# HilaManor/AudioEditingCode

Measured on AMD Instinct MI355X. Metric: edited-clips/sec (200-step inv+edit, 10 s@16 kHz), higher is better.
Workload: dtype f32

## Files before the change

audioeditingcode_amd/csrc/cg_params.h:

```cpp
#pragma once
#include "aed_common.h"

typedef float f32x16 __attribute__((ext_vector_type(16)));

struct CGParams {
    const float* A;
    const float* W;
    const float* bias;
    float* C;
    const float* res;
    const float* rowvec;
    float* ws;
    long long* dbg;
    const float* A2;
    int diag;
    int gm;
    int M, N, K;
    int lda, ldc, ldr, ld_rv;
    int IH, IW, OH, OW, Cin;
    int KH, KW, stride, pad_h, pad_w, dil_h, dil_w, up;
    int a_bs;
    int vIH, vIW;
    int o_mul, o_add, o_len, out_bs;
    int in_act, out_act, accumulate, ksplit;
    int rpb;
    int nchunks;
    int kgroup;
    float in_slope, out_p, out_div;
    int ln_mode;
    float ln_eps;
    int C1, lda2, a_bs2;
    int late_epilogue;
    int w_bs, vec_bs, vec_ld;
    int sm_group;
    float sm_scale;
    const float* kbias;
    int geglu;
    const unsigned char* Wq;
    const unsigned char* Wsc;
};

__device__ __forceinline__ float in_transform(float v, int act, float slope) {
    if (act == AED_ACT_SILU) return v / (1.0f + __expf(-v));
    if (act == AED_ACT_LEAKY) return v > 0.0f ? v : v * slope;
    return v;
}

__device__ __forceinline__ float gelu_exact(float g) { return 0.5f * g * (1.0f + erff(g * 0.70710678118654752440f)); }
__device__ __forceinline__ float glu_gate(float g, int kind) { return kind == 2 ? g / (1.0f + expf(-g)) : gelu_exact(g); }

__device__ __forceinline__ void store_out(const CGParams& p, int m, int n, float v) {
    int b = m / p.rpb;
    int q = m - b * p.rpb;
    int o = q * p.o_mul + p.o_add;
    if ((unsigned)o >= (unsigned)p.o_len) return;
    size_t row = (size_t)b * p.out_bs + o;
    if (p.bias) v += p.bias[n];
    if (p.rowvec && !p.ln_mode) v += p.rowvec[(size_t)b * p.ld_rv + n];
    if (p.res) v += p.res[row * p.ldr + n];
    v = aed_apply_act(v, p.out_act, p.out_p);
    float* dst = p.C + row * p.ldc + n;
    if (p.accumulate == 1) v += *dst;
    else if (p.accumulate == 2) v = (*dst + v) / p.out_div;
    *dst = v;
}

int cg_fill_params(const aed_op* op, CGParams& p, int bkt);
int launch_lin_gemm(const CGParams& p, int cfg, hipStream_t s);
```

audioeditingcode_amd/csrc/conv_gemm.hip:

```cpp
#include "cg_params.h"

template <int BM, int BN, int WROWS, int WCOLS, bool GENERIC, int DEPTH, int BKT, bool PLAIN>
__global__ __launch_bounds__(256, (BM * BN >= 128 * 128) ? 2 : 1) void conv_gemm_kernel(CGParams p) {
    constexpr int WM = BM / WROWS, WN = BN / WCOLS;
    constexpr int TM = WM / 32, TN = WN / 32;
    constexpr int LDS_LD = BKT + 4;
    constexpr int STAGE = (BM + BN) * LDS_LD;
    constexpr int TPR = BKT / 4;
    constexpr int RPP = 256 / TPR;
    constexpr int PA = BM / RPP, PB = BN / RPP;
    constexpr int NKB = BKT / 8;
    static_assert(WROWS * WCOLS == 4, "4 waves");
    static_assert(TM >= 1 && TN >= 1 && PA >= 1 && PB >= 1, "tile");

    __shared__ __attribute__((aligned(16))) float lds[2 * STAGE];

    const int tid = threadIdx.x;
    const int lane = tid & 63;
    const int wave = tid >> 6;
    const int wr = wave / WCOLS, wc = wave % WCOLS;
    int tile_x = blockIdx.x, tile_y = blockIdx.y;
    if (gridDim.z == 1) {
        const unsigned nx = gridDim.x, nwg = nx * gridDim.y;
        const unsigned orig = blockIdx.y * nx + blockIdx.x;
// ... 252 lines not shown
    if ((p.N & 3) == 0) {
        const size_t q4 = total >> 2;
        const float4* ws4 = reinterpret_cast<const float4*>(p.ws);
        for (size_t e4 = (size_t)blockIdx.x * 256 + threadIdx.x; e4 < q4; e4 += (size_t)gridDim.x * 256) {
            float4 v = ws4[e4];
#pragma unroll 4
            for (int z = 1; z < p.ksplit; ++z) {
                const float4 w = ws4[(size_t)z * q4 + e4];
                v.x += w.x; v.y += w.y; v.z += w.z; v.w += w.w;
            }
            const size_t e = e4 << 2;
            const int m = (int)(e / p.N);
            const int n = (int)(e - (size_t)m * p.N);
            store_out(p, m, n, v.x);
            store_out(p, m, n + 1, v.y);
            store_out(p, m, n + 2, v.z);
            store_out(p, m, n + 3, v.w);
        }
        return;
    }
    for (size_t e = (size_t)blockIdx.x * 256 + threadIdx.x; e < total; e += (size_t)gridDim.x * 256) {
        int m = (int)(e / p.N);
        int n = (int)(e - (size_t)m * p.N);
        float v = 0.f;
        for (int z = 0; z < p.ksplit; ++z) v += p.ws[(size_t)z * total + e];
        store_out(p, m, n, v);
    }
}

int cg_fill_params(const aed_op* op, CGParams& p, int bkt) {
    p.A = (const float*)op->p[0];
    p.W = (const float*)op->p[1];
    p.bias = (const float*)op->p[2];
    p.C = (float*)op->p[3];
    p.res = (const float*)op->p[4];
    p.rowvec = (const float*)op->p[5];
    p.ws = (float*)op->p[6];
    p.dbg = (op->flags & 1) ? (long long*)op->p[7] : nullptr;
    p.late_epilogue = (op->flags & 2) ? 1 : 0;
    const int32_t* i = op->i;
    p.M = i[0]; p.N = i[1]; p.K = i[2]; p.lda = i[3]; p.ldc = i[4]; p.ldr = i[5]; p.ld_rv = i[6];
    p.IH = i[7]; p.IW = i[8]; p.OH = i[9]; p.OW = i[10]; p.Cin = i[11]; p.KH = i[12]; p.KW = i[13];
    p.stride = i[14]; p.pad_h = i[15]; p.pad_w = i[16]; p.dil_h = i[17]; p.dil_w = i[18]; p.up = i[19];
    p.a_bs = i[20]; p.o_mul = i[21]; p.o_add = i[22]; p.o_len = i[23]; p.out_bs = i[24];
    p.in_act = i[25]; p.out_act = i[26]; p.accumulate = i[27]; p.ksplit = i[28];
    p.in_slope = op->f[0]; p.out_p = op->f[1]; p.out_div = op->f[2];
    p.ln_mode = i[31]; p.ln_eps = op->f[3];
    p.C1 = i[32]; p.lda2 = i[33]; p.a_bs2 = i[34]; p.geglu = i[35];
    p.A2 = (const float*)op->p[8];
    p.gm = 0;
    p.diag = (op->flags & 0x8000) ? 1 : 0;
    p.Wq = nullptr;
    p.Wsc = nullptr;
    p.sm_group = i[36]; p.w_bs = i[37]; p.vec_ld = i[38] > 0 ? i[38] : 1; p.vec_bs = i[39];
    p.sm_scale = op->f[4];
    p.kbias = (const float*)op->p[9];
    p.rpb = p.OH * p.OW;
    p.nchunks = (p.K + bkt - 1) / bkt;
    {
        const int g = bkt > 32 ? bkt : 32;
        p.kgroup = (p.KH * p.KW > 1 && p.Cin % g == 0 && p.Cin > g && !(op->flags & 32)) ? g : p.Cin;
    }
    p.vIH = p.IH << p.up;
    p.vIW = p.IW << p.up;
    if (p.up) {
        const int th = (p.OH - 1) * p.stride - 2 * p.pad_h + p.dil_h * (p.KH - 1) + 1;
        const int tw = (p.OW - 1) * p.stride - 2 * p.pad_w + p.dil_w * (p.KW - 1) + 1;
        if (th < p.vIH) p.vIH = th;
        if (tw < p.vIW) p.vIW = tw;
        AED_REQUIRE(p.vIH >= 2 * p.IH - 1 && p.vIW >= 2 * p.IW - 1, "conv_gemm: upsample target %dx%d too small for %dx%d",
                    th, tw, p.IH, p.IW);
    }
    AED_REQUIRE(p.A && p.W && p.C, "conv_gemm: null operand");
    AED_REQUIRE(p.M > 0 && p.N > 0 && p.K > 0, "conv_gemm: bad shape M=%d N=%d K=%d", p.M, p.N, p.K);
    AED_REQUIRE(p.K == p.KH * p.KW * p.Cin, "conv_gemm: K=%d != KH*KW*Cin=%d", p.K, p.KH * p.KW * p.Cin);
    AED_REQUIRE(p.rpb > 0 && p.M % p.rpb == 0, "conv_gemm: M=%d not a multiple of OH*OW=%d", p.M, p.rpb);
    AED_REQUIRE((long long)(p.M / p.rpb) * p.a_bs + (long long)p.IH * p.IW * p.lda < (1LL << 31) &&
                    (long long)p.N * p.K < (1LL << 31) &&
                    ((long long)(p.M / p.rpb) * p.out_bs + 1) * (long long)(p.ldc > p.ldr ? p.ldc : p.ldr) < (1LL << 31),
                "conv_gemm: operand exceeds the 32-bit element-offset range");
    if (p.ksplit < 1) p.ksplit = 1;
    if (p.ksplit > p.nchunks) p.ksplit = p.nchunks;
    if (p.ksplit > 1) AED_REQUIRE(p.ws != nullptr, "conv_gemm: split-K needs a workspace");
    if (p.ln_mode)
        AED_REQUIRE(p.ksplit == 1 && p.KH * p.KW == 1 && p.rowvec && p.bias && p.in_act == 0,
                    "conv_gemm: fused LayerNorm needs a 1-tap, unsplit GEMM with folded weights");
    if (p.C1 > 0)
        AED_REQUIRE(p.A2 && p.C1 % 64 == 0 && p.C1 < p.Cin && p.lda2 % 4 == 0 && ((uintptr_t)p.A2 % 16) == 0 &&
                        (long long)(p.M / p.rpb) * p.a_bs2 + (long long)p.IH * p.IW * p.lda2 < (1LL << 31),
                    "conv_gemm: bad two-source split C1=%d of Cin=%d", p.C1, p.Cin);
    if (p.geglu)
        AED_REQUIRE(p.ksplit == 1 && p.N % 64 == 0 && !p.res && p.out_act == 0 && p.accumulate == 0 && p.o_mul == 1 &&
                        p.o_add == 0 && p.o_len >= p.rpb && (p.ln_mode || !p.rowvec),
                    "conv_gemm: the GEGLU epilogue needs an unsplit GEMM with packed N %% 64 == 0 and a plain epilogue");
    return 0;
}

template <int BM, int BN, int WR, int WC, int DEPTH, int BKT>
static void launch_cfg(const CGParams& p, bool plain, hipStream_t s) {
    dim3 grid(aed_cdiv(p.N, BN), aed_cdiv(p.M, BM), p.ksplit);
    if (plain)
        hipLaunchKernelGGL((conv_gemm_kernel<BM, BN, WR, WC, false, DEPTH, BKT, true>), grid, dim3(256), 0, s, p);
    else
        hipLaunchKernelGGL((conv_gemm_kernel<BM, BN, WR, WC, false, DEPTH, BKT, false>), grid, dim3(256), 0, s, p);
}

// ... 83 lines not shown
```

audioeditingcode_amd/csrc/conv_gemm_x6.hip:

```cpp
#include "cg_params.h"

typedef __bf16 bf16x8 __attribute__((ext_vector_type(8)));
typedef __bf16 bf16x2 __attribute__((ext_vector_type(2)));
typedef float f32x2 __attribute__((ext_vector_type(2)));

int launch_conv_gemm_x6(const aed_op* op, hipStream_t s);

constexpr int X6_BK = 16;

__device__ __forceinline__ void x6_split_pair(float x0, float x1, unsigned& h, unsigned& m, unsigned& l) {
    h = __builtin_bit_cast(unsigned, __builtin_convertvector((f32x2){x0, x1}, bf16x2));
    float r0 = x0 - __uint_as_float(h << 16);
    float r1 = x1 - __uint_as_float(h & 0xffff0000u);
    asm volatile("" : "+v"(r0), "+v"(r1));
    m = __builtin_bit_cast(unsigned, __builtin_convertvector((f32x2){r0, r1}, bf16x2));
    float q0 = r0 - __uint_as_float(m << 16);
    float q1 = r1 - __uint_as_float(m & 0xffff0000u);
    asm volatile("" : "+v"(q0), "+v"(q1));
    l = __builtin_bit_cast(unsigned, __builtin_convertvector((f32x2){q0, q1}, bf16x2));
}

typedef unsigned u32x4 __attribute__((ext_vector_type(4)));
constexpr unsigned X6_OOB = 0x80000000u;

template <int G, int NM, int NV>
__device__ __forceinline__ void x6_hints() {
    if constexpr (G < NM) {
        constexpr int v = (NV * (G + 1)) / NM - (NV * G) / NM;
        if constexpr (v > 0) __builtin_amdgcn_sched_group_barrier(0x002, v, 0);
        __builtin_amdgcn_sched_group_barrier(0x008, 1, 0);
        x6_hints<G + 1, NM, NV>();
    }
}

template <int BM, int BN, int WROWS, int WCOLS, int DEPTH, bool PLAIN, int SCHED, int NTERMS, int BK = X6_BK>
__global__ __launch_bounds__(64 * WROWS * WCOLS, 2) void conv_gemm_x6_kernel(CGParams p) {
    constexpr int NT = 64 * WROWS * WCOLS;
    constexpr int WM = BM / WROWS, WN = BN / WCOLS;
    constexpr int TM = WM / 32, TN = WN / 32;
    constexpr int TPR = BK / 4;
    constexpr int RPP = NT / TPR;
    constexpr int PA = BM / RPP, PB = BN / RPP;
    constexpr int PQ = BK / 8;
    constexpr int X6_ROWQ = 3 * PQ + 1;
    constexpr int KB = BK / 16;
    constexpr int STAGE = (BM + BN) * X6_ROWQ;
    static_assert(BK == 16 || BK == 32, "chunk width");
    static_assert(TM >= 1 && TN >= 1 && PA >= 1 && PB >= 1, "tile");
    static_assert(BM % RPP == 0 && BN % RPP == 0, "loader passes");

    __shared__ uint4 lds[2 * STAGE];
    const unsigned nx = gridDim.x, ny = gridDim.y, bz = blockIdx.z, gz = gridDim.z;
    const unsigned orig = blockIdx.y * nx + blockIdx.x;

    const int tid = threadIdx.x;
    const int lane = tid & 63;
    const int wave = tid >> 6;
    const int wr = wave / WCOLS, wc = wave % WCOLS;
    int tile_y = (int)(orig / nx), tile_x = (int)(orig - (unsigned)tile_y * nx);
    if (gz == 1) {
        const unsigned nwg = nx * ny;
        const unsigned xcd = orig & 7u, q = nwg >> 3, r = nwg & 7u;
        const unsigned id = (xcd < r ? xcd * (q + 1) : r * (q + 1) + (xcd - r) * q) + (orig >> 3);
        if (p.gm > 1) {
            const unsigned per_group = (unsigned)p.gm * nx;
            const unsigned g = id / per_group, first = g * (unsigned)p.gm;
            const unsigned gsz = min((unsigned)p.gm, ny - first);
            const unsigned within = id - g * per_group;
            tile_x = (int)(within / gsz);
            tile_y = (int)(first + (within - (unsigned)tile_x * gsz));
        } else {
            tile_y = (int)(id / nx);
            tile_x = (int)(id - (unsigned)tile_y * nx);
        }
    }
    const int m0 = tile_y * BM;
    const int n0 = tile_x * BN;

    int kc_begin = 0, kc_end = p.nchunks;
    if (p.ksplit > 1) {
        const int per = (p.nchunks + p.ksplit - 1) / p.ksplit;
        kc_begin = (int)bz * per;
        kc_end = min(p.nchunks, kc_begin + per);
    }

    const int lrow = tid / TPR;
    const int lq = tid % TPR;
    const int lcol = lq * 4;

    int ay0[PA], ax0[PA];
    unsigned abase[PA], abase2[PA];
    bool avalid[PA];
#pragma unroll
    for (int q = 0; q < PA; ++q) {
        const int m = m0 + lrow + RPP * q;
        avalid[q] = m < p.M;
        const int mm = avalid[q] ? m : 0;
        int b = 0, r = mm, oy = mm, ox = 0;
        if (p.rpb != p.M || p.OW != 1) {
            b = mm / p.rpb;
            r = mm - b * p.rpb;
            oy = r / p.OW;
            ox = r - oy * p.OW;
        }
        ay0[q] = oy * p.stride - p.pad_h;
        ax0[q] = ox * p.stride - p.pad_w;
        abase[q] = (unsigned)b * (unsigned)p.a_bs + lcol;
        abase2[q] = (unsigned)b * (unsigned)p.a_bs2 + lcol;
    }
    unsigned wbase[PB];
    bool wvalid[PB];
#pragma unroll
    for (int q = 0; q < PB; ++q) {
        const int n = n0 + lrow + RPP * q;
        wvalid[q] = n < p.N;
        wbase[q] = (unsigned)(wvalid[q] ? n : 0) * (unsigned)p.K + lcol;
    }
    const int vIH = p.vIH, vIW = p.vIW;
    int pf_cg, pf_sub, pf_ty, pf_tx;
    const int gq = p.kgroup / BK;
    if (kc_begin == 0) {
        pf_cg = pf_sub = pf_ty = pf_tx = 0;
    } else {
        const int per_group = p.KH * p.KW * gq;
        const int g = kc_begin / per_group;
        const int rem = kc_begin - g * per_group;
        const int tap = rem / gq;
        pf_cg = g * p.kgroup;
        pf_sub = rem - tap * gq;
        pf_ty = tap / p.KW;
        pf_tx = tap - pf_ty * p.KW;
    }

    float4 rbuf_a[DEPTH][PA], rbuf_b[DEPTH][PB];
    float ln_s1[PA], ln_s2[PA];
#pragma unroll
    for (int q = 0; q < PA; ++q) { ln_s1[q] = 0.f; ln_s2[q] = 0.f; }

    const __amdgpu_buffer_rsrc_t srd_a = __builtin_amdgcn_make_buffer_rsrc((void*)p.A, 0, 0x7ffffff0, 0x00020000);
    const __amdgpu_buffer_rsrc_t srd_a2 = __builtin_amdgcn_make_buffer_rsrc((void*)(p.A2 ? p.A2 : p.A), 0, 0x7ffffff0, 0x00020000);
    const __amdgpu_buffer_rsrc_t srd_w = __builtin_amdgcn_make_buffer_rsrc((void*)p.W, 0, 0x7ffffff0, 0x00020000);
    auto as_f4 = [](u32x4 v) {
        return make_float4(__uint_as_float(v.x), __uint_as_float(v.y), __uint_as_float(v.z), __uint_as_float(v.w));
    };
    auto prefetch = [&](int kc, float4 (&ra)[PA], float4 (&rb)[PB]) {
        int c0 = pf_cg + pf_sub * BK;
        const int dy = pf_ty * p.dil_h, dx = pf_tx * p.dil_w;
        const unsigned k0 = (unsigned)((pf_ty * p.KW + pf_tx) * p.Cin + c0);
        pf_sub += 1;
        const bool wrap = pf_sub == gq;
        pf_sub = wrap ? 0 : pf_sub;
        pf_tx += wrap ? 1 : 0;
        const bool wrap2 = pf_tx == p.KW;
        pf_tx = wrap2 ? 0 : pf_tx;
        pf_ty += wrap2 ? 1 : 0;
        const bool wrap3 = pf_ty == p.KH;
        pf_ty = wrap3 ? 0 : pf_ty;
        pf_cg += wrap3 ? p.kgroup : 0;
        const bool second = p.C1 > 0 && c0 >= p.C1;
        c0 -= second ? p.C1 : 0;
        const unsigned ld = second ? (unsigned)p.lda2 : (unsigned)p.lda;
        const bool dead = kc >= kc_end;
#pragma unroll
        for (int q = 0; q < PA; ++q) {
            const int iy = ay0[q] + dy, ix = ax0[q] + dx;
            const bool ok = avalid[q] & ((unsigned)iy < (unsigned)vIH) & ((unsigned)ix < (unsigned)vIW) & !dead;
            const unsigned base = second ? abase2[q] : abase[q];
            const unsigned off = (base + (unsigned)((iy >> p.up) * p.IW + (ix >> p.up)) * ld + (unsigned)c0) * 4u;
            ra[q] = as_f4(__builtin_amdgcn_raw_buffer_load_b128(second ? srd_a2 : srd_a, ok ? off : X6_OOB, 0, 0));
        }
// ... 41 lines not shown
            }
            put_row(st, lrow + RPP * q, v);
        }
#pragma unroll
        for (int q = 0; q < PB; ++q) put_row(st, BM + lrow + RPP * q, rb[q], true);
    };

    f32x16 acc[TM][TN];
#pragma unroll
    for (int a = 0; a < TM; ++a)
#pragma unroll
        for (int b = 0; b < TN; ++b)
#pragma unroll
            for (int r = 0; r < 16; ++r) acc[a][b][r] = 0.f;

    const int fi = lane & 31;
    const int fh = lane >> 5;
    const int a_frag = (wr * WM + fi) * X6_ROWQ + fh;
    const int b_frag = (BM + wc * WN + fi) * X6_ROWQ + fh;

    bf16x8 af[TM][3], bw[TN][3];
    auto load_frags = [&](const uint4* st, int kb, bf16x8 (&fa)[TM][3], bf16x8 (&fb)[TN][3]) {
#pragma unroll
        for (int a = 0; a < TM; ++a)
#pragma unroll
            for (int pl = 0; pl < 3; ++pl)
                fa[a][pl] = __builtin_bit_cast(bf16x8, st[a_frag + a * 32 * X6_ROWQ + PQ * pl + 2 * kb]);
#pragma unroll
        for (int b = 0; b < TN; ++b)
#pragma unroll
            for (int pl = 0; pl < 3; ++pl)
                fb[b][pl] = __builtin_bit_cast(bf16x8, st[b_frag + b * 32 * X6_ROWQ + PQ * pl + 2 * kb]);
    };
    auto do_mfmas = [&](const bf16x8 (&fa)[TM][3], const bf16x8 (&fb)[TN][3]) {
        constexpr int TA[6] = {0, 2, 1, 0, 1, 0};
        constexpr int TB[6] = {2, 0, 1, 1, 0, 0};
#pragma unroll
        for (int t = 6 - NTERMS; t < 6; ++t)
#pragma unroll
            for (int a = 0; a < TM; ++a)
#pragma unroll
                for (int b = 0; b < TN; ++b)
                    acc[a][b] = __builtin_amdgcn_mfma_f32_32x32x16_bf16(fa[a][TA[t]], fb[b][TB[t]], acc[a][b], 0, 0, 0);
    };
    auto hints = [&]() {
        if constexpr (SCHED == 1) {
            constexpr int NM = TM * TN * NTERMS * KB;
            x6_hints<0, NM, NM * (((PA + PB) * 22 + 40 + NM - 1) / NM)>();
        }
    };

#pragma unroll
    for (int d = 0; d < DEPTH; ++d) prefetch(kc_begin + d, rbuf_a[d], rbuf_b[d]);
    stage_write(lds, rbuf_a[0], rbuf_b[0]);
    prefetch(kc_begin + DEPTH, rbuf_a[0], rbuf_b[0]);
    __syncthreads();
    int cur = 0;
    for (int kc0 = kc_begin; kc0 < kc_end; kc0 += DEPTH) {
#pragma unroll
        for (int d = 0; d < DEPTH; ++d) {
            const int kc = kc0 + d;
            const int sl = (d + 1) % DEPTH;
            load_frags(lds + cur * STAGE, 0, af, bw);
            stage_write(lds + (cur ^ 1) * STAGE, rbuf_a[sl], rbuf_b[sl]);
            prefetch(kc + 1 + DEPTH, rbuf_a[sl], rbuf_b[sl]);
            do_mfmas(af, bw);
            if constexpr (KB == 2) {
                bf16x8 af2[TM][3], bw2[TN][3];
                load_frags(lds + cur * STAGE, 1, af2, bw2);
                do_mfmas(af2, bw2);
            }
            hints();
            __syncthreads();
            cur ^= 1;
        }
    }

    float* ln_stat = reinterpret_cast<float*>(lds);
#include "cg_epilogue.h"
}

template <int BM, int BN, int WR, int WC, int DEPTH, bool DIAG, int BK = X6_BK>
static int x6_launch(const CGParams& p, bool plain, int sched, int terms, hipStream_t s) {
    dim3 grid(aed_cdiv(p.N, BN), aed_cdiv(p.M, BM), p.ksplit);
    dim3 block(64 * WR * WC);
#define X6_GO(PL, SC, NT_) hipLaunchKernelGGL((conv_gemm_x6_kernel<BM, BN, WR, WC, DEPTH, PL, SC, NT_, BK>), grid, block, 0, s, p)
    if (terms == 3) {
        if constexpr (DIAG) {
            if (plain) { X6_GO(true, 1, 3); return 0; }
        }
        AED_REQUIRE(false, "conv_gemm_x6: the three-term diagnostic exists for tiles 1 and 8 with a plain A operand");
    }
    if (!plain) X6_GO(false, 1, 6);
    else if (sched) X6_GO(true, 1, 6);
    else X6_GO(true, 0, 6);
#undef X6_GO
    return 0;
}

int launch_conv_gemm_x6(const aed_op* op, hipStream_t s) {
    const int32_t* i = op->i;
    const int Cin = i[11];
    int cfg = i[29];
    const long long batch = i[0] / (i[9] * i[10] > 0 ? i[9] * i[10] : 1);
    const bool fits = (Cin % X6_BK == 0) && (i[3] % 4 == 0) && ((uintptr_t)op->p[0] % 16 == 0) &&
                      ((uintptr_t)op->p[1] % 16 == 0) && cfg < 10 && cfg != 5 && cfg != 6 && cfg != 7 && i[36] == 0 &&
                      i[37] == 0 && i[38] <= 1 && i[39] == 0 &&
                      batch * i[20] + (long long)i[7] * i[8] * i[3] < (1LL << 29) && (long long)i[1] * i[2] < (1LL << 29) &&
                      (i[32] == 0 || batch * i[34] + (long long)i[7] * i[8] * i[33] < (1LL << 29));
    if (!fits) {
        if (cfg == 8 || cfg == 9) {
            aed_op fp32_op = *op;
            fp32_op.i[29] = 1;
            return launch_conv_gemm(&fp32_op, s);
        }
        return launch_conv_gemm(op, s);
    }
    const bool wide = (op->flags & 256) && (cfg == 8 || cfg == 9) && Cin % 32 == 0 && !(op->flags & 16);
    CGParams p;
    int rc = cg_fill_params(op, p, wide ? 32 : X6_BK);
    if (rc) return rc;
    if (p.ksplit > (p.K + 31) / 32) p.ksplit = (p.K + 31) / 32;
    if (cfg == 0) {
        const int cus = aed_num_cus();
        auto blocks = [&](int bm, int bn) { return (long)aed_cdiv(p.M, bm) * aed_cdiv(p.N, bn) * p.ksplit; };
        if (p.N >= 512 && p.N % 256 == 0 && blocks(128, 256) >= 2L * cus) cfg = 9;
        else if (blocks(256, 128) >= 2L * cus && p.N >= 128) cfg = 8;
        else if (blocks(128, 128) >= (long)cus && p.N >= 128) cfg = 1;
        else if (blocks(128, 64) >= 2L * cus) cfg = 2;
        else cfg = 4;
    }
    if (!(op->flags & 1024) && p.ksplit <= 1) {
        static const int BMs[10] = {0, 128, 128, 64, 64, 0, 0, 0, 256, 128}, BNs[10] = {0, 128, 64, 128, 64, 0, 0, 0, 128, 256};
        const int nx = aed_cdiv(p.N, BNs[cfg]), ny = aed_cdiv(p.M, BMs[cfg]);
        const int resident = ((aed_num_cus() >> ((op->flags >> 16) & 3)) / 8) * ((cfg == 8 || cfg == 9) ? 1 : 2);
        if (nx > 1 && ny > 1) {
            int g = 1;
            while (g * 2 <= ny && (long)(g * 2) * (g * 2) * BMs[cfg] <= (long)resident * BNs[cfg]) g *= 2;
            if (resident / g < nx) p.gm = g;
            if (op->flags & 0x3800) p.gm = 1 << ((op->flags >> 11) & 7);
        }
    }
    const bool plain = p.in_act == 0 && p.ln_mode == 0;
    const int sched = (op->flags & 8) ? 1 : 0;
    const int terms = (op->flags & 16) ? 3 : 6;
    if (p.geglu) AED_REQUIRE(cfg == 1 || cfg == 3 || cfg == 8 || cfg == 9, "conv_gemm_x6: the GEGLU epilogue needs 64-wide wave tiles (cfg %d)", cfg);
    switch (cfg) {
        case 1: rc = x6_launch<128, 128, 2, 2, 2, true>(p, plain, sched, terms, s); break;
        case 2: rc = x6_launch<128, 64, 2, 2, 2, false>(p, plain, sched, terms, s); break;
        case 3: rc = x6_launch<64, 128, 2, 2, 2, false>(p, plain, sched, terms, s); break;
        case 4: rc = x6_launch<64, 64, 2, 2, 2, false>(p, plain, sched, terms, s); break;
        case 8: rc = wide && terms == 6 ? x6_launch<256, 128, 4, 2, 2, false, 32>(p, plain, sched, terms, s)
                                        : x6_launch<256, 128, 4, 2, 2, true>(p, plain, sched, terms, s); break;
        case 9: rc = wide && terms == 6 ? x6_launch<128, 256, 2, 4, 2, false, 32>(p, plain, sched, terms, s)
                                        : x6_launch<128, 256, 2, 4, 2, false>(p, plain, sched, terms, s); break;
        default: AED_REQUIRE(false, "conv_gemm_x6: bad tile cfg %d", cfg);
    }
    if (rc) return rc;
    AED_CHECK_HIP(hipGetLastError());
    if (p.ksplit > 1) return launch_splitk_reduce(op, s);
    return 0;
}
```

audioeditingcode_amd/tape.py:

```python
import contextlib
import ctypes
import math
import threading

import torch

from . import _lib as L

CU_COUNT = 256


FORCE_BK = 0
ATTN_VARIANT = 0
ATTN_X6 = 1
GN_VARIANT = 0
GN_FORCE_SMALL = 0
GN_APPLY_BLOCKS_PER_CU = 8
LIN_MODE = 1
LATE_EPILOGUE = 0
WIDE_CHUNKS = 1
try:
    from .tile_table import TILE_TABLE
except ImportError:
    TILE_TABLE = {}
TILE_TABLE = dict(TILE_TABLE)
try:
    from .tile_table_dit import TILE_TABLE as _DIT_TABLE
    TILE_TABLE.update(_DIT_TABLE)
except ImportError:
    pass

REGIME_TABLES = {}
try:
    from .tile_table_cus128 import TILE_TABLE as _CUS128
    REGIME_TABLES["cus128"] = dict(_CUS128)
except ImportError:
    pass
try:
    from .tile_table_cus64 import TILE_TABLE as _CUS64
    REGIME_TABLES["cus64"] = dict(_CUS64)
except ImportError:
    pass
X6_TABLES = {}
for _reg, _mod in ((None, "tile_table_x6"), ("cus128", "tile_table_x6_cus128"), ("cus64", "tile_table_x6_cus64")):
    try:
        X6_TABLES[_reg] = dict(__import__(f"{__package__}.{_mod}", fromlist=["TILE_TABLE"]).TILE_TABLE)
    except ImportError:
        pass
for _reg, _mod in (("cus128", "tile_table_x6_cus128_b1"), ("cus64", "tile_table_x6_cus64_b1")):
    try:
        for _k, _v in __import__(f"{__package__}.{_mod}", fromlist=["TILE_TABLE"]).TILE_TABLE.items():
            X6_TABLES.setdefault(_reg, {}).setdefault(_k, _v)
    except ImportError:
        pass
REGIME_CUS = {"cus128": 128, "cus64": 64}
_regime = threading.local()


@contextlib.contextmanager
def tile_regime(name):
    if name is not None and name not in REGIME_TABLES:
        raise KeyError(f"unknown tile regime {name!r} (have {sorted(REGIME_TABLES)})")
    prev = getattr(_regime, "name", None)
    _regime.name = name
    try:
        yield
    finally:
        _regime.name = prev


ARITH_FLAGS = {"f32": 0, "bf16x6": 4 | 8, "fp8": 64 | 4 | 8}
FP8_ONLY = None
DEFAULT_ARITH = "f32"
# ... 1 lines not shown

@contextlib.contextmanager
def arith_mode(name):
    if name not in ARITH_FLAGS:
        raise KeyError(f"unknown arithmetic {name!r} (have {sorted(ARITH_FLAGS)})")
    prev = getattr(_regime, "arith", None)
    _regime.arith = name
    try:
        yield
    finally:
        _regime.arith = prev


def x6_tile(M, N, tile, ksplit, cus=None):
    cus = cus or CU_COUNT
    if tile == 1 and N >= 128:
        ks = max(ksplit, 1)
        if N >= 512 and N % 256 == 0 and math.ceil(M / 128) * (N // 256) * ks >= 2 * cus:
            return 9
        if math.ceil(M / 256) * math.ceil(N / 128) * ks >= 2 * cus:
            return 8
    return tile


FP8_PREQUANT = 1


def mx_quantized_weights(w, N, K):
    hit = getattr(w, "_aed_mxq", None)
    if hit is not None and hit[2] == (w.data_ptr(), N, K):
        return hit[0], hit[1]
    q = torch.empty((N, K), dtype=torch.uint8, device=w.device)
    sc = torch.empty((N, K // 32), dtype=torch.uint8, device=w.device)
    with torch.cuda.device(w.device):
        L.check(L.lib().aed_mx_quantize_rows(w.data_ptr(), q.data_ptr(), sc.data_ptr(), N, K, L.current_stream_ptr()),
                "aed_mx_quantize_rows")
    try:
        w._aed_mxq = (q, sc, (w.data_ptr(), N, K))
    except AttributeError:
        pass
    return q, sc


class Tape:
    def __init__(self, device):
        self.device = torch.device(device)
        self.ops = []
        self.meta = []
        self.keep = []
        self._arr = None
        self._ws_need = 0
        self._ws_ops = []
        self.ws = None
        self._graph = None

    def alloc(self, *shape, zero=False):
        t = (torch.zeros if zero else torch.empty)(shape, device=self.device, dtype=torch.float32)
        self.keep.append(t)
        return t

    def hold(self, t):
        self.keep.append(t)
        return t

    @staticmethod
    def _ptr(t):
        if t is None:
            return None
        if isinstance(t, int):
            return t
        return t.data_ptr()

    def _add(self, code, i=(), f=(), p=(), name="", flops=0, nbytes=0, flags=0, exec_flops=None):
        op = L.aed_op()
        op.code = code
        op.flags = flags
        for k, v in enumerate(i):
            op.i[k] = int(v)
        for k, v in enumerate(f):
            op.f[k] = float(v)
        for k, v in enumerate(p):
            op.p[k] = self._ptr(v)
            if torch.is_tensor(v):
                self.keep.append(v)
        self.ops.append(op)
        self.meta.append(dict(name=name or L.OP_NAMES[code], code=code, flops=flops, bytes=nbytes,
                              exec_flops=flops if exec_flops is None else exec_flops))
        self._arr = None
        return len(self.ops) - 1

    LIN_TILES = {10: (32, 32), 11: (32, 32), 12: (32, 32), 13: (32, 64), 14: (32, 64), 15: (64, 64), 16: (64, 32),
                 17: (64, 64), 18: (32, 32), 19: (32, 32)}

    @staticmethod
    def pick_tile(M, N, K, cus=None, vector_ok=True, geglu=False, lin_ok=True):
        cus = cus or CU_COUNT
        key = (M, N, K, int(bool(geglu)))
        reg = getattr(_regime, "name", None)
        for table in ((REGIME_TABLES[reg],) if reg else ()) + (TILE_TABLE,):
            hit = table.get(key)
            if hit is not None and (lin_ok or hit[0] < 10):
                return hit

        def blocks(bm, bn):
            return math.ceil(M / bm) * math.ceil(N / bn)
        if LIN_MODE and lin_ok and vector_ok and K % 32 == 0:
# ... 42 lines not shown
        M = B * OH * OW
        K = KH * KW * Cin
        lda = x.stride(-2) if lda is None else lda
        a_bs = IH * IW * lda if a_bs is None else a_bs
        ldc = out.stride(-2) if ldc is None else ldc
        if res is not None and ldr is None:
            ldr = res.stride(-2)
        o_len = OH * OW if o_len is None else o_len
        out_bs = OH * OW if out_bs is None else out_bs
        if x2 is not None:
            assert 0 < C1 < Cin and C1 % 64 == 0
            lda2 = x2.stride(-2) if lda2 is None else lda2
            a_bs2 = IH * IW * lda2 if a_bs2 is None else a_bs2
        vec_ok = (Cin % 32 == 0) and (lda % 4 == 0) and (x2 is None or lda2 % 4 == 0)
        lin_ok = vec_ok and accumulate == 0 and (x2 is None or C1 % 32 == 0)
        auto_tile, auto_split = self.pick_tile(M, N, K, vector_ok=vec_ok, geglu=bool(geglu), lin_ok=lin_ok)
        tile_forced = bool(tile)
        tile = tile or auto_tile
        ksplit = ksplit or auto_split
        if w_bs or vec_bs or sm_group or vec_ld != 1:
            assert lin_ok and KH * KW == 1 and (OH * OW) % 64 == 0, "per-batch operands need the lin_gemm path"
            if tile < 10:
                tile = 10
        if tile >= 10:
            ksplit = 1
        ln_mode = 0
        if ln_rowsum is not None:
            assert KH * KW == 1 and rowvec is None and bias is not None and vec_ok
            ln_mode, rowvec, ksplit = 1, ln_rowsum, 1
        i = [M, N, K, lda, ldc, ldr or 0, ld_rv, IH, IW, OH, OW, Cin, KH, KW, stride, pad_h, pad_w, dil_h, dil_w, up,
             a_bs, o_mul, o_add, o_len, out_bs, in_act, out_act, accumulate, ksplit, tile, FORCE_BK, ln_mode,
             C1 if x2 is not None else 0, lda2 or 0, a_bs2 or 0, int(geglu), sm_group, w_bs, vec_ld, vec_bs]
        n_out = N // 2 if geglu else N
        flags = 2 if LATE_EPILOGUE else 0
        arith = ARITH_FLAGS[getattr(_regime, "arith", None) or DEFAULT_ARITH]
        if arith & 64 and FP8_ONLY is not None and not FP8_ONLY(name):
            arith = ARITH_FLAGS["bf16x6"]
        x6_ok = arith and vec_ok and B * a_bs + IH * IW * lda < (1 << 29) and N * K < (1 << 29) and \
            (x2 is None or B * a_bs2 + IH * IW * lda2 < (1 << 29)) and not (w_bs or vec_bs or sm_group or vec_ld != 1) and \
            self._ptr(x) % 16 == 0 and self._ptr(w) % 16 == 0
        swept = X6_TABLES.get(getattr(_regime, "name", None), {}).get((M, N, K, int(bool(geglu)))) if x6_ok else None
        if swept is not None and not tile_forced and (swept[0] >= 100 or lin_ok):
            t, ks = swept
            if t >= 100:
                flags |= arith
                t -= 100
            ksplit = 1 if (t >= 10 or ln_mode) else max(ks, 1)
            i[28], i[29] = ksplit, t
        elif x6_ok and tile in (1, 2, 3, 4):
            flags |= arith
            i[29] = x6_tile(M, N, tile, ksplit)
        if flags & 4 and i[29] in (8, 9) and KH * KW > 1 and Cin % 32 == 0 and (x2 is None or C1 % 32 == 0) and WIDE_CHUNKS:
            flags |= 256
        if flags & 4:
            lane_cus = REGIME_CUS.get(getattr(_regime, "name", None), CU_COUNT)
            flags |= {1: 0, 2: 1, 4: 2, 8: 3}.get(max(1, CU_COUNT // max(lane_cus, 1)), 0) << 16
        idx = self._add(L.OP_CONV_GEMM, i, [in_slope, out_p, out_div, ln_eps, sm_scale],
                        [x, w, bias, out, res, rowvec, None, None, x2, kbias], name=name,
                        flops=2 * M * N * K if alg_flops is None else alg_flops, exec_flops=2 * M * N * K,
                        nbytes=4 * (B * IH * IW * Cin + N * K + M * n_out), flags=flags)
        f8_fits = x6_ok and Cin % 64 == 0 and lda % 4 == 0 and (x2 is None or C1 % 64 == 0) and i[29] in (0, 1, 2, 3, 4, 8, 9) \
            and not (i[36] or i[37] or i[39]) and i[38] <= 1
        if flags & 64 and FP8_PREQUANT and f8_fits and kbias is None and torch.is_tensor(w) and w.is_cuda:
            q, sc = mx_quantized_weights(w, N, K)
            self.keep += [q, sc]
            self.ops[idx].p[7], self.ops[idx].p[9] = q.data_ptr(), sc.data_ptr()
            self.ops[idx].flags |= 128
        if ksplit > 1:
            self._ws_need = max(self._ws_need, ksplit * M * N)
            self._ws_ops.append(idx)
        return out

    def linear(self, x, w, bias, out, *, M, K, N, lda=None, **kw):
        lda = x.stride(-2) if lda is None else lda
        return self.conv(x, w, bias, out, B=1, IH=M, IW=1, Cin=K, OH=M, OW=1, N=N, lda=lda, a_bs=0, **kw)

    TILE_BM = {1: 128, 2: 128, 3: 64, 4: 64, 5: 128, 6: 32}

    def groupnorm(self, x, gamma, beta, out, *, B, HW, C, G=32, eps=1e-5, act=0, variant=None, x2=None, C1=0,
                  name="gn"):
        ldx = x.stride(-2)
        ldy = out.stride(-2)
        ldx2 = x2.stride(-2) if x2 is not None else 0
        C1 = C1 if x2 is not None else 0
        variant = GN_VARIANT if variant is None else variant
        sliver = (C // G) < 8 and HW >= 2048 and not GN_FORCE_SMALL
        odd = (C // G) % 4 != 0 or ldx % 4 != 0 or ldy % 4 != 0 or (x2 is not None and (C1 % 4 != 0 or ldx2 % 4 != 0))
        if odd or (HW * (C // G) <= 65536 and B * G >= 32 and B * HW * C <= (1 << 22) and not sliver):
            self._add(L.OP_GN_SMALL, [B, HW, C, G, ldx, ldy, act, variant, C1, ldx2], [eps], [x, gamma, beta, out, x2],
                      name=name + ".gn1", nbytes=12 * B * HW * C)
            return out
        s_rpc = max(4, math.ceil(HW / 32))
        s_chunks = math.ceil(HW / s_rpc)
        a_target = max(1, (GN_APPLY_BLOCKS_PER_CU * CU_COUNT) // max(1, B))
        a_rpc = max(16, math.ceil(HW / a_target))
        a_chunks = math.ceil(HW / a_rpc)
        part = self.alloc(B, s_chunks, G, 2)
        nb = 4 * B * HW * C
        self._add(L.OP_GN_STATS, [B, HW, C, G, ldx, s_rpc, s_chunks, C1, ldx2], [], [x, part, x2],
                  name=name + ".stats", nbytes=nb)
        self._add(L.OP_GN_APPLY, [B, HW, C, G, ldx, a_rpc, s_chunks, act, ldy, a_chunks, C1, ldx2], [eps],
                  [x, part, gamma, beta, out, x2], name=name + ".apply", nbytes=2 * nb)
        return out

    def attention(self, q, k, v, out, *, B, H, Nq, Nk, D, ldq, ldk, ldv, ldo, bsq, bsk, bsv, bso, scale,
                  bias=None, ld_bias=0, variant=None, name="attn"):
        variant = ATTN_VARIANT if variant is None else variant
        arith = ARITH_FLAGS[getattr(_regime, "arith", None) or DEFAULT_ARITH] if ATTN_X6 else 0
        if arith & 4 and variant == 0 and D in (32, 48, 64) and Nk > 64 and \
                self._ptr(q) % 16 == 0 and self._ptr(k) % 16 == 0 and \
                math.ceil(Nq / 128) * H * B >= REGIME_CUS.get(getattr(_regime, "name", None), CU_COUNT):
            variant = 3
        self._add(L.OP_ATTENTION, [B, H, Nq, Nk, D, ldq, ldk, ldv, ldo, ld_bias, bsq, bsk, bsv, bso, variant], [scale],
                  [q, k, v, bias, out], name=name, flops=4 * B * H * Nq * Nk * D,
                  nbytes=4 * B * H * D * (2 * Nq + 2 * Nk), flags=arith & 4)
        return out

    def xattn_fold(self, kv, xq, xs, xo, G, gs, VOt, *, B, Lk, H, C, D, name="xattn_fold"):
        self._add(L.OP_XATTN_FOLD, [B, Lk, H, C, D, kv.stride(-2)], [], [kv, xq, xs, xo, G, gs, VOt], name=name,
                  flops=0, nbytes=4 * (2 * B * H * Lk * C))

    def copy2d(self, src, dst, *, rows, cols, ld_src=None, ld_dst=None, state=None, idx_off=0, idx_mul=0,
               idx_stride=0, coef=None, c_mul=0, c_off=0, c_stride=0, c_col=0, name="copy"):
# ... 49 lines not shown
        return y

    def advance(self, state, by=1):
        self._add(L.OP_ADVANCE, [by], [], [state], name="advance")

    def step(self, code, *, xts, zs, eps_u, eps_c, cfg, coef, state, out, numel, P, T, s_imm=0, v_pred=0, flag=1,
             cfg_scalar=1.0, c_imm=(0, 0, 0, 0, 0), s_mul=1, s_off=0, name="step"):
        self._add(code, [numel & 0xFFFFFFFF, numel >> 32, P, T, s_imm, v_pred, flag, s_mul, s_off],
                  [cfg_scalar, *c_imm],
                  [xts, zs, eps_u, eps_c, cfg, coef, state, out], name=name, nbytes=4 * numel * 6)

    def step_variants(self, *, cur, zs, eps, cfg, coef, state, numel, a, Z, v_pred=0, out=None, s_imm=0,
                      c_imm=(0, 0, 0, 0, 0), s_mul=1, s_off=0, name="step_variants"):
        has_noise = int(zs is not None)
        self._add(L.OP_REVERSE_STEP_VARIANTS, [numel & 0xFFFFFFFF, numel >> 32, a, Z if has_noise else 0, s_imm, v_pred,
                                               has_noise, s_mul, s_off],
                  [0.0, *c_imm], [cur, zs, eps, None, cfg, coef, state, out], name=name,
                  nbytes=4 * numel * (4 * a + has_noise))

    def rotary(self, x, cos, sin, *, M, N, H, D, R, ld=None, nsec=2, sec_stride=None, name="rotary"):
        ld = x.stride(-2) if ld is None else ld
        sec_stride = H * D if sec_stride is None else sec_stride
        self._add(L.OP_ROTARY, [M, N, H, D, R, ld, nsec, sec_stride], [], [x, cos, sin], name=name,
                  nbytes=8 * M * nsec * H * R)
        return x

    def snake(self, x, out, a, inv_b, *, rows, C, name="snake"):
        self._add(L.OP_SNAKE, [rows & 0xFFFFFFFF, rows >> 32, C, x.stride(-2), out.stride(-2)], [], [x, out, a, inv_b],
                  name=name, nbytes=8 * rows * C)
        return out

    def sa_step(self, mode, *, xts, zs, v_u, v_c, coef, state, hist, numel, T, out=None, extra=None, fix=1, cfg=1.0,
                s_imm=0, s_mul=1, s_off=0, name="sa_step"):
        self._add(L.OP_SA_STEP, [numel & 0xFFFFFFFF, numel >> 32, mode, T, s_imm, int(fix), s_mul, s_off], [cfg],
                  [xts, zs, v_u, v_c, coef, state, hist, out, extra], name=name, nbytes=4 * numel * 7)

    def gauss_sample(self, moments, noise, out, *, rows, C, name="gauss_sample"):
        self._add(L.OP_GAUSS_SAMPLE, [rows & 0xFFFFFFFF, rows >> 32, C, moments.stride(-2)], [], [moments, noise, out],
                  name=name, nbytes=16 * rows * C)
        return out

    def reflect_pad(self, src, dst, *, B, N, pad, ldd, name="reflect_pad"):
        self._add(L.OP_REFLECT_PAD, [B, N, pad, ldd], [], [src, dst], name=name, nbytes=8 * B * N)

    def magnitude(self, ft, mag, *, F, cut, ld_ft, ld_mag, name="magnitude"):
        self._add(L.OP_MAGNITUDE, [F, cut, ld_ft, ld_mag], [], [ft, mag], name=name, nbytes=4 * F * (2 * cut + ld_mag))

    def finalize(self):
        if self._arr is None:
            if self._ws_need and (self.ws is None or self.ws.numel() < self._ws_need):
                self.ws = torch.empty(self._ws_need, device=self.device, dtype=torch.float32)
            for idx in self._ws_ops:
                self.ops[idx].p[6] = self.ws.data_ptr()
            self._arr = (L.aed_op * len(self.ops))(*self.ops)
        return self._arr

    @property
    def flops(self):
        return sum(m["flops"] for m in self.meta)

    @property
    def exec_flops(self):
        return sum(m["exec_flops"] for m in self.meta)

    def run(self, start=0, end=None):
        arr = self.finalize()
        end = len(self.ops) if end is None else end
        if end <= start:
            return
        sub = ctypes.cast(ctypes.byref(arr, start * ctypes.sizeof(L.aed_op)), ctypes.POINTER(L.aed_op))
        L.check(L.lib().aed_tape_run(sub, end - start, L.current_stream_ptr()), "aed_tape_run")

    def profile(self):
        arr = self.finalize()
        ms = (ctypes.c_float * len(self.ops))()
        L.check(L.lib().aed_tape_profile(arr, len(self.ops), L.current_stream_ptr(), ms), "aed_tape_profile")
        return list(ms)

    def capture(self):
        lib = L.lib()
        sp = L.current_stream_ptr()
        L.check(lib.aed_graph_begin(sp), "aed_graph_begin")
        try:
            self.run()
        finally:
            g = ctypes.c_void_p()
            rc = lib.aed_graph_end(sp, ctypes.byref(g))
        L.check(rc, "aed_graph_end")
        self._graph = g
        return g

    def replay(self):
        L.check(L.lib().aed_graph_launch(self._graph, L.current_stream_ptr()), "aed_graph_launch")

    def __del__(self):
        try:
            if self._graph is not None:
                L.lib().aed_graph_destroy(self._graph)
        except Exception:
            pass
```

Measured before the change: 0.9007.

## Add persistent work-stealing x6 GEMM kernel with per-XCD atomic tile counters

Adds a persistent variant of the x6 conv-GEMM kernel for big 256x128/128x256 tile configs whose tile count exceeds the resident workgroup slots. Workgroups claim further tiles from per-XCD atomic counters, steal from other XCDs once their own queue is empty, and prefetch the next tile's first chunks before the epilogue. This targets wave-quantization tails and launch imbalance across XCDs. In exchange it adds atomic traffic, a per-op counter slab with reset logic, and extra register pressure from the tile-loop state.

```diff
diff --git a/audioeditingcode_amd/csrc/cg_params.h b/audioeditingcode_amd/csrc/cg_params.h
--- a/audioeditingcode_amd/csrc/cg_params.h
+++ b/audioeditingcode_amd/csrc/cg_params.h
@@ -38,6 +38,8 @@
     int geglu;
     const unsigned char* Wq;
     const unsigned char* Wsc;
+    int pnx, pny;
+    unsigned* tctr;
 };
 
 __device__ __forceinline__ float in_transform(float v, int act, float slope) {
diff --git a/audioeditingcode_amd/csrc/conv_gemm.hip b/audioeditingcode_amd/csrc/conv_gemm.hip
--- a/audioeditingcode_amd/csrc/conv_gemm.hip
+++ b/audioeditingcode_amd/csrc/conv_gemm.hip
@@ -328,6 +328,8 @@
     p.diag = (op->flags & 0x8000) ? 1 : 0;
     p.Wq = nullptr;
     p.Wsc = nullptr;
+    p.pnx = p.pny = 0;
+    p.tctr = nullptr;
     p.sm_group = i[36]; p.w_bs = i[37]; p.vec_ld = i[38] > 0 ? i[38] : 1; p.vec_bs = i[39];
     p.sm_scale = op->f[4];
     p.kbias = (const float*)op->p[9];
diff --git a/audioeditingcode_amd/csrc/conv_gemm_x6.hip b/audioeditingcode_amd/csrc/conv_gemm_x6.hip
--- a/audioeditingcode_amd/csrc/conv_gemm_x6.hip
+++ b/audioeditingcode_amd/csrc/conv_gemm_x6.hip
@@ -33,7 +33,7 @@
     }
 }
 
-template <int BM, int BN, int WROWS, int WCOLS, int DEPTH, bool PLAIN, int SCHED, int NTERMS, int BK = X6_BK>
+template <int BM, int BN, int WROWS, int WCOLS, int DEPTH, bool PLAIN, int SCHED, int NTERMS, int BK = X6_BK, bool PERSIST = false>
 __global__ __launch_bounds__(64 * WROWS * WCOLS, 2) void conv_gemm_x6_kernel(CGParams p) {
     constexpr int NT = 64 * WROWS * WCOLS;
     constexpr int WM = BM / WROWS, WN = BN / WCOLS;
@@ -50,32 +50,33 @@
     static_assert(BM % RPP == 0 && BN % RPP == 0, "loader passes");
 
     __shared__ uint4 lds[2 * STAGE];
-    const unsigned nx = gridDim.x, ny = gridDim.y, bz = blockIdx.z, gz = gridDim.z;
+    const unsigned nx = PERSIST ? (unsigned)p.pnx : gridDim.x, ny = PERSIST ? (unsigned)p.pny : gridDim.y;
+    const unsigned bz = blockIdx.z, gz = gridDim.z;
     const unsigned orig = blockIdx.y * nx + blockIdx.x;
 
     const int tid = threadIdx.x;
     const int lane = tid & 63;
     const int wave = tid >> 6;
     const int wr = wave / WCOLS, wc = wave % WCOLS;
-    int tile_y = (int)(orig / nx), tile_x = (int)(orig - (unsigned)tile_y * nx);
-    if (gz == 1) {
-        const unsigned nwg = nx * ny;
-        const unsigned xcd = orig & 7u, q = nwg >> 3, r = nwg & 7u;
-        const unsigned id = (xcd < r ? xcd * (q + 1) : r * (q + 1) + (xcd - r) * q) + (orig >> 3);
+    const unsigned nwg = nx * ny, xq = nwg >> 3, xr = nwg & 7u;
+    auto x_first = [&](unsigned x) { return x < xr ? x * (xq + 1) : xr * (xq + 1) + (x - xr) * xq; };
+    auto tile_of = [&](unsigned id, int& tx, int& ty) {
         if (p.gm > 1) {
             const unsigned per_group = (unsigned)p.gm * nx;
             const unsigned g = id / per_group, first = g * (unsigned)p.gm;
             const unsigned gsz = min((unsigned)p.gm, ny - first);
             const unsigned within = id - g * per_group;
-            tile_x = (int)(within / gsz);
-            tile_y = (int)(first + (within - (unsigned)tile_x * gsz));
+            tx = (int)(within / gsz);
+            ty = (int)(first + (within - (unsigned)tx * gsz));
         } else {
-            tile_y = (int)(id / nx);
-            tile_x = (int)(id - (unsigned)tile_y * nx);
-        }
-    }
-    const int m0 = tile_y * BM;
-    const int n0 = tile_x * BN;
+            ty = (int)(id / nx);
+            tx = (int)(id - (unsigned)ty * nx);
+        }
+    };
+    int tile_y = (int)(orig / nx), tile_x = (int)(orig - (unsigned)tile_y * nx);
+    if (PERSIST || gz == 1) tile_of(x_first(orig & 7u) + (orig >> 3), tile_x, tile_y);
+    int m0 = tile_y * BM;
+    int n0 = tile_x * BN;
 
     int kc_begin = 0, kc_end = p.nchunks;
     if (p.ksplit > 1) {
@@ -91,31 +92,34 @@
     int ay0[PA], ax0[PA];
     unsigned abase[PA], abase2[PA];
     bool avalid[PA];
-#pragma unroll
-    for (int q = 0; q < PA; ++q) {
-        const int m = m0 + lrow + RPP * q;
-        avalid[q] = m < p.M;
-        const int mm = avalid[q] ? m : 0;
-        int b = 0, r = mm, oy = mm, ox = 0;
-        if (p.rpb != p.M || p.OW != 1) {
-            b = mm / p.rpb;
-            r = mm - b * p.rpb;
-            oy = r / p.OW;
-            ox = r - oy * p.OW;
-        }
-        ay0[q] = oy * p.stride - p.pad_h;
-        ax0[q] = ox * p.stride - p.pad_w;
-        abase[q] = (unsigned)b * (unsigned)p.a_bs + lcol;
-        abase2[q] = (unsigned)b * (unsigned)p.a_bs2 + lcol;
-    }
     unsigned wbase[PB];
     bool wvalid[PB];
-#pragma unroll
-    for (int q = 0; q < PB; ++q) {
-        const int n = n0 + lrow + RPP * q;
-        wvalid[q] = n < p.N;
-        wbase[q] = (unsigned)(wvalid[q] ? n : 0) * (unsigned)p.K + lcol;
-    }
+    auto tile_rows = [&](int tm0, int tn0) {
+#pragma unroll
+        for (int q = 0; q < PA; ++q) {
+            const int m = tm0 + lrow + RPP * q;
+            avalid[q] = m < p.M;
+            const int mm = avalid[q] ? m : 0;
+            int b = 0, r = mm, oy = mm, ox = 0;
+            if (p.rpb != p.M || p.OW != 1) {
+                b = mm / p.rpb;
+                r = mm - b * p.rpb;
+                oy = r / p.OW;
+                ox = r - oy * p.OW;
+            }
+            ay0[q] = oy * p.stride - p.pad_h;
+            ax0[q] = ox * p.stride - p.pad_w;
+            abase[q] = (unsigned)b * (unsigned)p.a_bs + lcol;
+            abase2[q] = (unsigned)b * (unsigned)p.a_bs2 + lcol;
+        }
+#pragma unroll
+        for (int q = 0; q < PB; ++q) {
+            const int n = tn0 + lrow + RPP * q;
+            wvalid[q] = n < p.N;
+            wbase[q] = (unsigned)(wvalid[q] ? n : 0) * (unsigned)p.K + lcol;
+        }
+    };
+    tile_rows(m0, n0);
     const int vIH = p.vIH, vIW = p.vIW;
     int pf_cg, pf_sub, pf_ty, pf_tx;
     const int gq = p.kgroup / BK;
@@ -263,39 +267,122 @@
 
 #pragma unroll
     for (int d = 0; d < DEPTH; ++d) prefetch(kc_begin + d, rbuf_a[d], rbuf_b[d]);
-    stage_write(lds, rbuf_a[0], rbuf_b[0]);
-    prefetch(kc_begin + DEPTH, rbuf_a[0], rbuf_b[0]);
-    __syncthreads();
-    int cur = 0;
-    for (int kc0 = kc_begin; kc0 < kc_end; kc0 += DEPTH) {
-#pragma unroll
-        for (int d = 0; d < DEPTH; ++d) {
-            const int kc = kc0 + d;
-            const int sl = (d + 1) % DEPTH;
-            load_frags(lds + cur * STAGE, 0, af, bw);
-            stage_write(lds + (cur ^ 1) * STAGE, rbuf_a[sl], rbuf_b[sl]);
-            prefetch(kc + 1 + DEPTH, rbuf_a[sl], rbuf_b[sl]);
-            do_mfmas(af, bw);
-            if constexpr (KB == 2) {
-                bf16x8 af2[TM][3], bw2[TN][3];
-                load_frags(lds + cur * STAGE, 1, af2, bw2);
-                do_mfmas(af2, bw2);
+    [[maybe_unused]] unsigned claim = 0;
+    for (;;) {
+        if constexpr (PERSIST) {
+            if (tid == 0) claim = atomicAdd(p.tctr + (orig & 7u), 1u);
+        }
+        stage_write(lds, rbuf_a[0], rbuf_b[0]);
+        prefetch(kc_begin + DEPTH, rbuf_a[0], rbuf_b[0]);
+        __syncthreads();
+        int cur = 0;
+        for (int kc0 = kc_begin; kc0 < kc_end; kc0 += DEPTH) {
+#pragma unroll
+            for (int d = 0; d < DEPTH; ++d) {
+                const int kc = kc0 + d;
+                const int sl = (d + 1) % DEPTH;
+                load_frags(lds + cur * STAGE, 0, af, bw);
+                stage_write(lds + (cur ^ 1) * STAGE, rbuf_a[sl], rbuf_b[sl]);
+                prefetch(kc + 1 + DEPTH, rbuf_a[sl], rbuf_b[sl]);
+                do_mfmas(af, bw);
+                if constexpr (KB == 2) {
+                    bf16x8 af2[TM][3], bw2[TN][3];
+                    load_frags(lds + cur * STAGE, 1, af2, bw2);
+                    do_mfmas(af2, bw2);
+                }
+                hints();
+                __syncthreads();
+                cur ^= 1;
             }
-            hints();
+        }
+
+        float* ln_stat = reinterpret_cast<float*>(lds);
+        [[maybe_unused]] int next = -1, next_m0 = 0, next_n0 = 0;
+        if constexpr (PERSIST) {
+            __shared__ int x6_next;
+            if (wave == 0) {
+                const unsigned G = gridDim.x;
+                auto x_size = [&](unsigned x) { return xq + (x < xr ? 1u : 0u); };
+                auto x_wgs = [&](unsigned x) { return (G + 7u - x) >> 3; };
+                const unsigned own = orig & 7u, got = __shfl(claim, 0);
+                int t = -1;
+                if (x_wgs(own) + got < x_size(own)) {
+                    t = (int)(x_first(own) + x_wgs(own) + got);
+                } else {
+                    for (;;) {
+                        const unsigned x = (own + (unsigned)lane) & 7u;
+                        bool left = false;
+                        if (lane < 8) left = x_wgs(x) + __hip_atomic_load(p.tctr + x, __ATOMIC_RELAXED, __HIP_MEMORY_SCOPE_AGENT) < x_size(x);
+                        const unsigned long long bal = __ballot(left);
+                        if (bal == 0) break;
+                        const int l = __ffsll((long long)bal) - 1;
+                        unsigned c = 0;
+                        if (lane == l) c = atomicAdd(p.tctr + x, 1u);
+                        c = __shfl(c, l);
+                        const unsigned xs = (own + (unsigned)l) & 7u;
+                        if (x_wgs(xs) + c < x_size(xs)) {
+                            t = (int)(x_first(xs) + x_wgs(xs) + c);
+                            break;
+                        }
+                    }
+                }
+                if (tid == 0) x6_next = t;
+            }
             __syncthreads();
-            cur ^= 1;
-        }
-    }
-
-    float* ln_stat = reinterpret_cast<float*>(lds);
+            next = x6_next;
+            if (next >= 0) {
+                int tx, ty;
+                tile_of((unsigned)next, tx, ty);
+                next_m0 = ty * BM;
+                next_n0 = tx * BN;
+                tile_rows(next_m0, next_n0);
+                pf_cg = pf_sub = pf_ty = pf_tx = 0;
+#pragma unroll
+                for (int d = 0; d < DEPTH; ++d) prefetch(d, rbuf_a[d], rbuf_b[d]);
+            }
+        }
 #include "cg_epilogue.h"
+        if constexpr (!PERSIST) {
+            break;
+        } else {
+            if (next < 0) break;
+            __syncthreads();
+            m0 = next_m0;
+            n0 = next_n0;
+#pragma unroll
+            for (int a = 0; a < TM; ++a)
+#pragma unroll
+                for (int b = 0; b < TN; ++b)
+#pragma unroll
+                    for (int r = 0; r < 16; ++r) acc[a][b][r] = 0.f;
+#pragma unroll
+            for (int q = 0; q < PA; ++q) { ln_s1[q] = 0.f; ln_s2[q] = 0.f; }
+        }
+    }
+    if constexpr (PERSIST) {
+        if (tid == 0 && atomicAdd(p.tctr + 8, 1u) == gridDim.x - 1) {
+#pragma unroll
+            for (int x = 0; x < 9; ++x) __hip_atomic_store(p.tctr + x, 0u, __ATOMIC_RELAXED, __HIP_MEMORY_SCOPE_AGENT);
+        }
+    }
 }
 
 template <int BM, int BN, int WR, int WC, int DEPTH, bool DIAG, int BK = X6_BK>
-static int x6_launch(const CGParams& p, bool plain, int sched, int terms, hipStream_t s) {
+static int x6_launch(const CGParams& p, bool plain, int sched, int terms, int persist_wgs, hipStream_t s) {
     dim3 grid(aed_cdiv(p.N, BN), aed_cdiv(p.M, BM), p.ksplit);
     dim3 block(64 * WR * WC);
 #define X6_GO(PL, SC, NT_) hipLaunchKernelGGL((conv_gemm_x6_kernel<BM, BN, WR, WC, DEPTH, PL, SC, NT_, BK>), grid, block, 0, s, p)
+    if constexpr (BK == X6_BK) {
+      if (persist_wgs > 0) {
+        CGParams pp = p;
+        pp.pnx = (int)grid.x;
+        pp.pny = (int)grid.y;
+        const dim3 pgrid((unsigned)min((long)persist_wgs, (long)grid.x * grid.y));
+        if (plain) hipLaunchKernelGGL((conv_gemm_x6_kernel<BM, BN, WR, WC, DEPTH, true, 1, 6, BK, true>), pgrid, block, 0, s, pp);
+        else hipLaunchKernelGGL((conv_gemm_x6_kernel<BM, BN, WR, WC, DEPTH, false, 1, 6, BK, true>), pgrid, block, 0, s, pp);
+        return 0;
+      }
+    }
     if (terms == 3) {
         if constexpr (DIAG) {
             if (plain) { X6_GO(true, 1, 3); return 0; }
@@ -355,16 +442,22 @@
     const bool plain = p.in_act == 0 && p.ln_mode == 0;
     const int sched = (op->flags & 8) ? 1 : 0;
     const int terms = (op->flags & 16) ? 3 : 6;
+    int persist_wgs = 0;
+    if ((op->flags & 16384) && op->p[9] && p.ksplit <= 1 && sched && terms == 6 && !wide) {
+        AED_REQUIRE((uintptr_t)op->p[9] % 64 == 0, "conv_gemm_x6: the counter slab must be 64-byte aligned");
+        p.tctr = (unsigned*)op->p[9];
+        persist_wgs = (aed_num_cus() >> ((op->flags >> 16) & 3)) * ((cfg == 8 || cfg == 9) ? 1 : 2);
+    }
     if (p.geglu) AED_REQUIRE(cfg == 1 || cfg == 3 || cfg == 8 || cfg == 9, "conv_gemm_x6: the GEGLU epilogue needs 64-wide wave tiles (cfg %d)", cfg);
     switch (cfg) {
-        case 1: rc = x6_launch<128, 128, 2, 2, 2, true>(p, plain, sched, terms, s); break;
-        case 2: rc = x6_launch<128, 64, 2, 2, 2, false>(p, plain, sched, terms, s); break;
-        case 3: rc = x6_launch<64, 128, 2, 2, 2, false>(p, plain, sched, terms, s); break;
-        case 4: rc = x6_launch<64, 64, 2, 2, 2, false>(p, plain, sched, terms, s); break;
-        case 8: rc = wide && terms == 6 ? x6_launch<256, 128, 4, 2, 2, false, 32>(p, plain, sched, terms, s)
-                                        : x6_launch<256, 128, 4, 2, 2, true>(p, plain, sched, terms, s); break;
-        case 9: rc = wide && terms == 6 ? x6_launch<128, 256, 2, 4, 2, false, 32>(p, plain, sched, terms, s)
-                                        : x6_launch<128, 256, 2, 4, 2, false>(p, plain, sched, terms, s); break;
+        case 1: rc = x6_launch<128, 128, 2, 2, 2, true>(p, plain, sched, terms, persist_wgs, s); break;
+        case 2: rc = x6_launch<128, 64, 2, 2, 2, false>(p, plain, sched, terms, persist_wgs, s); break;
+        case 3: rc = x6_launch<64, 128, 2, 2, 2, false>(p, plain, sched, terms, persist_wgs, s); break;
+        case 4: rc = x6_launch<64, 64, 2, 2, 2, false>(p, plain, sched, terms, persist_wgs, s); break;
+        case 8: rc = wide && terms == 6 ? x6_launch<256, 128, 4, 2, 2, false, 32>(p, plain, sched, terms, persist_wgs, s)
+                                        : x6_launch<256, 128, 4, 2, 2, true>(p, plain, sched, terms, persist_wgs, s); break;
+        case 9: rc = wide && terms == 6 ? x6_launch<128, 256, 2, 4, 2, false, 32>(p, plain, sched, terms, persist_wgs, s)
+                                        : x6_launch<128, 256, 2, 4, 2, false>(p, plain, sched, terms, persist_wgs, s); break;
         default: AED_REQUIRE(false, "conv_gemm_x6: bad tile cfg %d", cfg);
     }
     if (rc) return rc;
diff --git a/audioeditingcode_amd/tape.py b/audioeditingcode_amd/tape.py
--- a/audioeditingcode_amd/tape.py
+++ b/audioeditingcode_amd/tape.py
@@ -19,6 +19,9 @@
 LIN_MODE = 1
 LATE_EPILOGUE = 0
 WIDE_CHUNKS = 1
+X6_PERSIST = 1
+X6_TILE_SHAPES = {1: (128, 128), 2: (128, 64), 3: (64, 128), 4: (64, 64), 8: (256, 128), 9: (128, 256)}
+X6_CTR_WORDS = 16
 try:
     from .tile_table import TILE_TABLE
 except ImportError:
@@ -126,6 +129,8 @@
         self._ws_need = 0
         self._ws_ops = []
         self.ws = None
+        self._ctr_ops = []
+        self.ctr = None
         self._graph = None
 
     def alloc(self, *shape, zero=False):
@@ -274,9 +279,16 @@
             i[29] = x6_tile(M, N, tile, ksplit)
         if flags & 4 and i[29] in (8, 9) and KH * KW > 1 and Cin % 32 == 0 and (x2 is None or C1 % 32 == 0) and WIDE_CHUNKS:
             flags |= 256
+        persist = False
         if flags & 4:
             lane_cus = REGIME_CUS.get(getattr(_regime, "name", None), CU_COUNT)
             flags |= {1: 0, 2: 1, 4: 2, 8: 3}.get(max(1, CU_COUNT // max(lane_cus, 1)), 0) << 16
+            bm_bn = X6_TILE_SHAPES.get(i[29]) if i[29] in (8, 9) else None
+            if X6_PERSIST and bm_bn and ksplit <= 1 and not flags & (16 | 64 | 256):
+                slots = (CU_COUNT >> ((flags >> 16) & 3)) * (1 if i[29] in (8, 9) else 2)
+                persist = math.ceil(M / bm_bn[0]) * math.ceil(N / bm_bn[1]) > slots
+                if persist:
+                    flags |= 16384
         idx = self._add(L.OP_CONV_GEMM, i, [in_slope, out_p, out_div, ln_eps, sm_scale],
                         [x, w, bias, out, res, rowvec, None, None, x2, kbias], name=name,
                         flops=2 * M * N * K if alg_flops is None else alg_flops, exec_flops=2 * M * N * K,
@@ -291,6 +303,8 @@
         if ksplit > 1:
             self._ws_need = max(self._ws_need, ksplit * M * N)
             self._ws_ops.append(idx)
+        if persist:
+            self._ctr_ops.append(idx)
         return out
 
     def linear(self, x, w, bias, out, *, M, K, N, lda=None, **kw):
@@ -446,6 +460,11 @@
                 self.ws = torch.empty(self._ws_need, device=self.device, dtype=torch.float32)
             for idx in self._ws_ops:
                 self.ops[idx].p[6] = self.ws.data_ptr()
+            if self._ctr_ops and (self.ctr is None or self.ctr.numel() < X6_CTR_WORDS * len(self._ctr_ops)):
+                self.ctr = torch.zeros(X6_CTR_WORDS * len(self._ctr_ops), device=self.device, dtype=torch.int32)
+                self.keep.append(self.ctr)
+            for k, idx in enumerate(self._ctr_ops):
+                self.ops[idx].p[9] = self.ctr.data_ptr() + 4 * X6_CTR_WORDS * k
             self._arr = (L.aed_op * len(self.ops))(*self.ops)
         return self._arr
 
```

New measurement: 0.9387, median of 6. 4.2% higher.
